# ethz-asl/multipoint

Measured on AMD Instinct MI355X. Metric: image-pairs/sec (detect+desc+match) @ 480x640, higher is better.
Workload: dtype f32

## Files before the change

multipoint_amd/csrc/conv_wino43.hip:

```cpp
#include "mp_common.h"
#include "mp_device.h"
#include "mp_tile.h"

#include <algorithm>
#include <type_traits>

MP_TIMING_TABLE(g_timing_q, 256 * 8, mp_debug_read_timing_wino43)
MP_TIMING_HEIGHT(g_timing_q_sel, 480, mp_debug_select_height_wino43)

namespace {

constexpr int NPIX = 18 * 34;
constexpr int UC4 = 4;
constexpr int VB4 = UC4 * 32 * 36;
constexpr int UB4 = UC4 * 64 * 36;
constexpr int NRB = (NPIX + 63) / 64;
constexpr int RB4 = NRB * 64 * 4;
constexpr int SW4 = 8 * 36 * 2;


template <int LEAD = 0>
__device__ __forceinline__ void dma16(const float* sbase, unsigned voff_bytes, unsigned lds_byte)
{
    lds_dma<4, LEAD, 0>(sbase, voff_bytes, lds_byte);
}

template <bool POOL, bool BNF, int TC4, bool F1, bool SPLIT = false, bool VIN = false>
__global__ __launch_bounds__(512, 2) void conv_wino43_kernel(const ConvParams p)
{
    static_assert(!(F1 && SPLIT), "the fused first block is never split");
    static_assert(!(VIN && (F1 || SPLIT)), "pre-transformed input: plain launches only");
    constexpr int TR4 = 32 / TC4;
    constexpr int OY = 4 * TR4, OX = 4 * TC4;
    constexpr int PY = OY + 2, PX = OX + 2;
    static_assert(PY * PX == NPIX, "item shape");
    __shared__ __attribute__((aligned(16))) float Vs[(VIN ? 4 : 2) * VB4];
    __shared__ __attribute__((aligned(16))) float Us[2 * UB4];
    __shared__ __attribute__((aligned(16))) float raw[VIN ? 256 : 3 * RB4 + 256];
    __shared__ __attribute__((aligned(16))) float scr[VIN ? 4 : 8 * SW4];
    __shared__ __attribute__((aligned(16))) float prm[(POOL && !SPLIT ? 6 : 3) * 64];

    const int tid = threadIdx.x;
    const int lane = tid & 63;
    const int wave = __builtin_amdgcn_readfirstlane(tid >> 6);
    const int tb = wave & 1, cb = wave >> 1;
    const int NC = SPLIT ? (p.cin / UC4) >> p.ks_shift : p.cin / UC4;

    const XcdRange xr = xcd_range(p.nitems, p.xcd_shift);
    const int stride = xr.stride, item_end = xr.item_end;
    int item = xr.item;
    if (item >= item_end) return;

    struct Where { int slice, img, y0, x0, tile; const float* in_base; };
    auto decode = [&](int it) __attribute__((always_inline)) -> Where {
        Where w{};
        const int tile = (int)udiv((unsigned)it, p.magic_slices, (unsigned)p.nslices);
        w.slice = it - tile * p.nslices;
        w.tile = tile;
        const int trow = (int)udiv((unsigned)tile, p.magic_tx, (unsigned)p.tiles_x);
        const int tx = tile - trow * p.tiles_x;
        const int bi = (int)udiv((unsigned)trow, p.magic_ty, (unsigned)p.tiles_y);
        const int ty = trow - bi * p.tiles_y;
        w.img = p.img_list ? p.img_list[bi] : bi;
        w.y0 = ty * OY; w.x0 = tx * OX;
        w.in_base = p.in_planar ? p.in + (long long)w.img * (p.cin / 4) * p.H * p.W * 4
                                : p.in + (long long)w.img * p.H * p.W * p.in_cstride + p.in_coff;
        if constexpr (SPLIT)
            w.in_base += (long long)((w.slice & ((1 << p.ks_shift) - 1)) * NC) * (p.in_planar ? (long long)p.H * p.W * 4 : UC4);
        return w;
    };

    const int pix_stride = p.in_planar ? 4 : p.in_cstride;
    const long long unit_stride = p.in_planar ? (long long)p.H * p.W * 4 : UC4;
    const int x_shift = p.in_planar == MP_LAYOUT_XPLANAR ? 2 : 0, x_mask = p.in_planar == MP_LAYOUT_XPLANAR ? 3 : 0;
    const int row_stride = p.W * pix_stride;
    auto pixel_off = [&](int y, int x) __attribute__((always_inline)) -> int {
        return y * row_stride + (x >> x_shift) * pix_stride + (x & x_mask) * p.W;
    };
    unsigned rvoff[2];
    bool roff_rel = false;
    auto raw_offsets = [&](const Where& w) __attribute__((always_inline)) -> const float* {
        const bool interior = (w.y0 >= 1) && (w.y0 + OY < p.H) && (w.x0 >= 1) && (w.x0 + OX < p.W);
        if (interior) {
            if (!roff_rel) {
#pragma unroll
                for (int j = 0; j < 2; ++j) {
                    const int f = (wave + 8 * j) * 64 + lane;
                    const int py = f / PX, px = f - py * PX;
                    rvoff[j] = (f < NPIX) ? (unsigned)pixel_off(py, px + x_mask) * 4u : 0u;
                }
                roff_rel = true;
            }
            return w.in_base + pixel_off(w.y0 - 1, w.x0 - 1 - x_mask);
        }
        roff_rel = false;
#pragma unroll
        for (int j = 0; j < 2; ++j) {
            const int f = (wave + 8 * j) * 64 + lane;
            const int py = f / PX, px = f - py * PX;
            unsigned off = 0;
            if (f < NPIX) {
                const int gy = reflect_clamp(w.y0 + py - 1, p.H), gx = reflect_clamp(w.x0 + px - 1, p.W);
                off = (unsigned)pixel_off(gy, gx) * 4u;
            }
            rvoff[j] = off;
        }
        return w.in_base;
    };
    const unsigned raw_lds = lds_addr(raw), us_lds = lds_addr(Us);
    const unsigned raw_m0 = raw_lds + (unsigned)wave * 1024u;
    const unsigned raw_dummy = raw_lds + 3u * RB4 * 4u;
    auto raw_dma = [&](const float* src, unsigned boff_bytes, int j) __attribute__((always_inline)) {
        const unsigned dst = j == 0 ? raw_m0 + boff_bytes : (wave + 8 < NRB ? raw_m0 + 8192u + boff_bytes : raw_dummy);
        dma16(src, rvoff[j], dst);
    };
    int u_first, u_cnt;
    if constexpr (F1) {
        constexpr int cnt_[8] = {3, 3, 6, 6, 4, 4, 5, 5}, first_[8] = {0, 3, 14, 20, 6, 10, 26, 31};
        u_cnt = 3; u_first = 0;
#pragma unroll
        for (int w = 0; w < 8; ++w) { u_cnt = wave == w ? cnt_[w] : u_cnt; u_first = wave == w ? first_[w] : u_first; }
    } else {
        u_cnt = wave < 4 ? 5 : 4; u_first = wave < 4 ? 5 * wave : 20 + 4 * (wave - 4);
    }
    auto u_dma_site = [&](const float* ub, int buf, int site) __attribute__((always_inline)) {
        if constexpr (VIN) {
#pragma unroll
            for (int i = 3 * site; i < (site ? 5 : 3); ++i) {
                int b = wave + 8 * i;
                b = b < 36 ? b : 35;
                dma16(ub + b * 256, (unsigned)lane * 16u, us_lds + (unsigned)(buf * UB4 + b * 256) * 4u);
            }
            return;
        }
#pragma unroll
        for (int k = 3 * site; k < 3 * site + 3; ++k)
            if (k < u_cnt) {
                const int b = u_first + k;
                dma16<1>(ub + b * 256, (unsigned)lane * 16u, us_lds + (unsigned)(buf * UB4 + b * 256) * 4u);
            }
    };
    auto u_ptr = [&](int slice) __attribute__((always_inline)) -> const float* {
        return p.wpack + (long long)slice * NC * UB4;
    };
    auto load_prm = [&](int vslice) __attribute__((always_inline)) {
        const int slice = SPLIT ? vslice >> p.ks_shift : vslice;
        if (tid < 64) {
            const float sc = p.scale[slice * 64 + tid];
            prm[tid] = p.bias[slice * 64 + tid]; prm[128 + tid] = p.shift[slice * 64 + tid];
            if constexpr (POOL && !SPLIT) {
                const bool neg = sc < 0.f;
                prm[64 + tid] = fabsf(sc); prm[192 + tid] = neg ? -1.f : 1.f;
                prm[256 + tid] = __int_as_float(neg ? (int)0x80000000 : 0); prm[320 + tid] = __int_as_float(neg ? 0 : 0x7fffffff);
            } else {
                prm[64 + tid] = sc;
            }
        }
    };

    const int win = tid >> 3, sub = tid & 7;
    const int w_tile = win >> 1, w_cp = win & 1;
    const int w_ty = w_tile / TC4, w_tx = w_tile % TC4;
    const int sub6 = sub < 6 ? sub : 5;
    const int p1_read = ((4 * w_ty) * PX + 4 * w_tx + sub6) * 4 + 2 * w_cp;
    float* const myscr = scr + wave * SW4 + (win & 7) * 72;
    const unsigned scr_w = lds_addr(myscr + sub6 * 2);
    const int p2_write = (2 * w_cp * 32 + w_tile) * 36 + 6 * sub6;
    f32x2 td[6], tr[6];
    typedef const __attribute__((address_space(3))) f32x2* lds_pair_ptr;
    const unsigned p1_base = lds_addr(raw) + (unsigned)p1_read * 4u;
    unsigned p1_a = p1_base, p1_b = p1_base + 4u * PX * 16u;
    auto tf_pass1 = [&]() __attribute__((always_inline)) {
#pragma unroll
        for (int i = 0; i < 4; ++i) td[i] = reinterpret_cast<lds_pair_ptr>(p1_a)[i * PX * 2];
#pragma unroll
        for (int i = 4; i < 6; ++i) td[i] = reinterpret_cast<lds_pair_ptr>(p1_b)[(i - 4) * PX * 2];
    };
    auto tf_pass1b = [&](unsigned next_byte) __attribute__((always_inline)) {
        bt6(td, tr);
        p1_a = p1_base + next_byte; p1_b = p1_base + 4u * PX * 16u + next_byte;
    };
    auto tf_pass1w = [&](int k) __attribute__((always_inline)) {
        unsigned long long save;
        if (k == 0)
            asm volatile("s_mov_b64 %0, exec\n\ts_and_b64 exec, exec, %4\n\tds_write2_b64 %1, %2, %3 offset0:0 offset1:6\n\ts_mov_b64 exec, %0"
                         : "=&s"(save) : "v"(scr_w), "v"(tr[0]), "v"(tr[1]), "s"(0x3F3F3F3F3F3F3F3Full) : "memory");
        else if (k == 1)
            asm volatile("s_mov_b64 %0, exec\n\ts_and_b64 exec, exec, %4\n\tds_write2_b64 %1, %2, %3 offset0:12 offset1:18\n\ts_mov_b64 exec, %0"
                         : "=&s"(save) : "v"(scr_w), "v"(tr[2]), "v"(tr[3]), "s"(0x3F3F3F3F3F3F3F3Full) : "memory");
        else
            asm volatile("s_mov_b64 %0, exec\n\ts_and_b64 exec, exec, %4\n\tds_write2_b64 %1, %2, %3 offset0:24 offset1:30\n\ts_mov_b64 exec, %0"
                         : "=&s"(save) : "v"(scr_w), "v"(tr[4]), "v"(tr[5]), "s"(0x3F3F3F3F3F3F3F3Full) : "memory");
    };
    auto tf_pass2 = [&]() __attribute__((always_inline)) {
#pragma unroll
        for (int j = 0; j < 6; ++j) td[j] = *reinterpret_cast<const f32x2*>(&myscr[(sub6 * 6 + j) * 2]);
    };
    const unsigned p2_addr = lds_addr(Vs) + (unsigned)p2_write * 4u;
    auto tf_pass2b = [&]() __attribute__((always_inline)) {
        bt6(td, tr);
    };
    auto tf_pass2w = [&](int buf, int k) __attribute__((always_inline)) {
        const unsigned a0 = p2_addr + (unsigned)buf * (VB4 * 4u), a1 = a0 + 32u * 36u * 4u;
        const int j = 2 * k;
        unsigned long long save;
#define MPQ_VST(O0, O1)                                                                                                        \
        asm volatile("s_mov_b64 %0, exec\n\ts_and_b64 exec, exec, %7\n\tds_write2_b32 %1, %2, %3 offset0:" #O0 " offset1:" #O1   \
                     "\n\tds_write2_b32 %4, %5, %6 offset0:" #O0 " offset1:" #O1 "\n\ts_mov_b64 exec, %0"                        \
                     : "=&s"(save) : "v"(a0), "v"(tr[j][0]), "v"(tr[j + 1][0]), "v"(a1), "v"(tr[j][1]), "v"(tr[j + 1][1]),       \
                       "s"(0x3F3F3F3F3F3F3F3Full) : "memory")
        if (k == 0) MPQ_VST(0, 1);
        else if (k == 1) MPQ_VST(2, 3);
        else MPQ_VST(4, 5);
#undef MPQ_VST
    };

    const int a_base = ((lane >> 4) * 64 + cb * 16 + (lane & 15)) * 36;
    const int b_base = ((lane >> 4) * 32 + tb * 16 + (lane & 15)) * 36;
    f32x4 af[3], bf[3];

    constexpr int IW1 = PX + 2, IH1 = PY + 2;
    constexpr int IPB = 768;
    static_assert(!F1 || (IH1 * IW1 <= IPB && 2 * IPB + 16 * 4 + 16 * 4 * 12 <= RB4), "F1: patches + parameters + weights must fit the third raw buffer");
    const unsigned ip_lds = raw_lds + 2u * RB4 * 4u;
    const unsigned bst_lds = ip_lds + 2u * IPB * 4u;
    const unsigned w1_lds = bst_lds + 16u * 4u * 4u;
    typedef const __attribute__((address_space(3))) float* lds_f32_ptr;
    typedef const __attribute__((address_space(3))) f32x4* lds_f32x4_ptr;
    typedef __attribute__((address_space(3))) f32x4* lds_f32x4_wptr;
    unsigned pg_x[2] = {0u, 0u}, pg_w[2] = {0u, 0u};
    bool pg_rel = false;
    int pc_par = 0;
    auto prod_offsets = [&](const Where& w) __attribute__((always_inline)) {
        const bool interior = (w.y0 >= 1) && (w.y0 + OY < p.H) && (w.x0 >= 1) && (w.x0 + OX < p.W);
#pragma unroll
        for (int j = 0; j < 2; ++j) {
            const int f = (wave + 8 * j) * 64 + lane;
            const int fc = f < NPIX ? f : NPIX - 1;
            const int py = fc / PX, px = fc - py * PX;
            int oy = py, ox = px;
            if (!interior) {
                oy = reflect_clamp(w.y0 + py - 1, p.H) - w.y0 + 1; ox = reflect_clamp(w.x0 + px - 1, p.W) - w.x0 + 1;
                oy = min(max(oy, 0), IH1 - 3); ox = min(max(ox, 0), IW1 - 3);
            }
            pg_x[j] = ip_lds + (unsigned)(pc_par * IPB + oy * IW1 + ox) * 4u;
            pg_w[j] = (unsigned)f * 16u;
        }
        pg_rel = interior;
    };
    auto patch_dma = [&](const Where& w, int par) __attribute__((always_inline)) {
        const float* const im = p.img + (long long)w.img * p.H * p.W;
#pragma unroll
        for (int j = 0; j < 2; ++j) {
            if (wave * 64 + 512 * j >= IH1 * IW1) continue;
            const int q = min(tid + 512 * j, IH1 * IW1 - 1);
            const int r = q / IW1, c = q - r * IW1;
            const unsigned off = (unsigned)(reflect_clamp(w.y0 - 2 + r, p.H) * p.W + reflect_clamp(w.x0 - 2 + c, p.W)) * 4u;
            lds_dma<1, 0, 0>(im, off, ip_lds + (unsigned)(par * IPB + wave * 64 + 512 * j) * 4u);
        }
    };
    int pc_unit = 0, pc_next_item = item + stride;
    unsigned pc_wv = w1_lds + (unsigned)(lane & 3) * 48u;
    unsigned pc_bv = bst_lds;
    float px_[9];
    f32x4 pw_[3], pd_;
    auto gather_x = [&](float (&x)[9], const int j) __attribute__((always_inline)) {
        const lds_f32_ptr xp = reinterpret_cast<lds_f32_ptr>(pg_x[j]);
#pragma unroll
        for (int t = 0; t < 9; ++t) x[t] = xp[(t / 3) * IW1 + (t % 3)];
    };
    auto prod_step = [&](const int k, const unsigned wbuf, const int j, const float (&x)[9]) __attribute__((always_inline)) {
        const lds_f32x4_ptr wp = reinterpret_cast<lds_f32x4_ptr>(pc_wv);
        const lds_f32x4_ptr bp = reinterpret_cast<lds_f32x4_ptr>(pc_bv);
        if (k == 0) {
            pd_ = bp[0];
            pw_[0] = wp[0]; pw_[1] = wp[1]; pw_[2] = wp[2];
        } else if (k <= 9) {
            pd_ = __builtin_amdgcn_mfma_f32_4x4x1f32(pw_[(k - 1) >> 2][(k - 1) & 3], x[k - 1], pd_, 0, 0, 0);
        } else {
            const f32x4 v = {relu_bits(pd_[0]), relu_bits(pd_[1]), relu_bits(pd_[2]), relu_bits(pd_[3])};
            *reinterpret_cast<lds_f32x4_wptr>(raw_lds + wbuf + pg_w[j]) = v;
        }
    };
    auto produce = [&](const unsigned wbuf, const int j) __attribute__((always_inline)) {
        if (j == 0) {
#pragma unroll
            for (int k = 0; k <= 10; ++k) prod_step(k, wbuf, 0, px_);
        } else {
            float qx[9];
            gather_x(qx, 1);
#pragma unroll
            for (int k = 0; k <= 10; ++k) prod_step(k, wbuf, 1, qx);
        }
    };
    auto prod_advance = [&]() __attribute__((always_inline)) {
        pc_wv += 4u * 12u * 4u; pc_bv += 4u * 4u;
        if (++pc_unit == NC) {
            pc_unit = 0;
            pc_wv -= (unsigned)NC * 4u * 12u * 4u; pc_bv -= (unsigned)NC * 4u * 4u;
            if (pc_next_item < item_end) {
                const Where w = decode(pc_next_item);
                pc_par ^= 1;
                if (!(pg_rel && (w.y0 >= 1) && (w.y0 + OY < p.H) && (w.x0 >= 1) && (w.x0 + OX < p.W))) prod_offsets(w);
                else {
                    const unsigned flip = pc_par ? (unsigned)IPB * 4u : 0u - (unsigned)IPB * 4u;
                    pg_x[0] += flip; pg_x[1] += flip;
                }
                gather_x(px_, 0);
                pc_next_item += stride;
            }
        }
    };

    const unsigned vs_lds = lds_addr(Vs);
    auto v_dma = [&](const float* vsrc, int slot, int i) __attribute__((always_inline)) {
        const int b = wave + 8 * i;
        const unsigned dst = b < 18 ? vs_lds + (unsigned)(slot * VB4 + b * 256) * 4u : lds_addr(raw);
        dma16(vsrc + (b < 18 ? b : 17) * 256, (unsigned)lane * 16u, dst);
    };
    const float* vcur = nullptr;
    int v_chunk = 0, v_next_item = item + stride;
    auto v_advance = [&]() __attribute__((always_inline)) {
        vcur += VB4;
        if (++v_chunk == NC) {
            v_chunk = 0;
            if (v_next_item < item_end) {
                vcur = p.vglobal + (long long)decode(v_next_item).tile * NC * VB4;
                v_next_item += stride;
            } else {
                vcur -= (long long)NC * VB4;
            }
        }
    };

    Where cur = decode(item);
    if constexpr (F1) {
        for (int f = tid; f < 16 * 4 * 12; f += 512) {
            const int ch = f / 12, t = f - ch * 12;
            (raw + 2 * RB4 + 2 * IPB + 16 * 4)[f] = t < 9 ? p.w1[t * 64 + ch] : 0.f;
        }
        if (tid < 64) (raw + 2 * RB4 + 2 * IPB)[tid] = p.b1[tid];
        patch_dma(cur, 0);
        if (item + stride < item_end) patch_dma(decode(item + stride), 1);
        prod_offsets(cur);
        dma_wait();
        __syncthreads();
        gather_x(px_, 0);
        produce(0u, 0); if (wave + 8 < NRB) produce(0u, 1);
        prod_advance();
        produce(RB4 * 4u, 0); if (wave + 8 < NRB) produce(RB4 * 4u, 1);
        prod_advance();
    }
    const float* rbase = (F1 || VIN) ? p.in : raw_offsets(cur);
    const float* rsrc = rbase;
    Where ld_item = cur;
    int ld_chunk = 0;
    int ld_next_item = item + stride;
    auto ld_advance = [&]() __attribute__((always_inline)) {
        rsrc += unit_stride;
        if (++ld_chunk == NC) {
            ld_chunk = 0;
            if (ld_next_item < item_end) {
                ld_item = decode(ld_next_item);
                rbase = raw_offsets(ld_item);
                ld_next_item += stride;
            }
            rsrc = rbase;
        }
    };
    const float* up = u_ptr(cur.slice);
    if constexpr (VIN) {
        vcur = p.vglobal + (long long)cur.tile * NC * VB4;
#pragma unroll
        for (int u = 0; u < 3; ++u) {
            v_dma(vcur, u, 0); v_dma(vcur, u, 1); v_dma(vcur, u, 2);
            v_advance();
        }
    } else if constexpr (!F1) {
        raw_dma(rsrc, 0u, 0); raw_dma(rsrc, 0u, 1); ld_advance();
        raw_dma(rsrc, RB4 * 4u, 0); raw_dma(rsrc, RB4 * 4u, 1); ld_advance();
        raw_dma(rsrc, 2u * RB4 * 4u, 0); raw_dma(rsrc, 2u * RB4 * 4u, 1); ld_advance();
    }
    unsigned rd_byte = 0u, rt_byte = RB4 * 4u;
    u_dma_site(up, 0, 0); u_dma_site(up, 0, 1);
    u_dma_site(up + UB4, 1, 0); u_dma_site(up + UB4, 1, 1);
    load_prm(cur.slice);
    dma_wait();
    __syncthreads();
    if constexpr (!VIN) {
        tf_pass1(); tf_pass1b(RB4 * 4u); tf_pass1w(0); tf_pass1w(1); tf_pass1w(2); tf_pass2(); tf_pass2b();
        tf_pass2w(0, 0); tf_pass2w(0, 1); tf_pass2w(0, 2);
        asm volatile("s_waitcnt lgkmcnt(0)" ::: "memory");
        __syncthreads();
    }
    af[0] = *reinterpret_cast<const f32x4*>(&Us[a_base]);
    bf[0] = *reinterpret_cast<const f32x4*>(&Vs[b_base]);
    af[1] = *reinterpret_cast<const f32x4*>(&Us[a_base + 4]);
    bf[1] = *reinterpret_cast<const f32x4*>(&Vs[b_base + 4]);

    const f32x4 zero4 = {0.f, 0.f, 0.f, 0.f};
    int cur_par = 0;
#ifdef MP_TIMING
    unsigned long long tsum[8] = {0, 0, 0, 0, 0, 0, 0, 0};
    const bool t_on = ((POOL ? p.H : -p.H) == g_timing_q_sel);
#endif
    for (;;) {
        MP_CLOCK(t_item);
        f32x4 acc[36];
        const int item_next = item + stride;
        const bool has_next = item_next < item_end;
        const int next_slice = has_next ? (int)(item_next - (int)udiv((unsigned)item_next, p.magic_slices, (unsigned)p.nslices) * p.nslices)
                                        : cur.slice;
        const float* unext = u_ptr(next_slice);
        auto tf_at = [&](const int g, const int e, const int vb) __attribute__((always_inline)) {
            constexpr int S[2][8][2] = {
                {{0, 2}, {2, 2}, {2, 3}, {3, 1}, {3, 2}, {5, 2}, {5, 3}, {6, 1}},
                {{0, 2}, {2, 2}, {2, 3}, {3, 1}, {3, 2}, {4, 3}, {5, 1}, {6, 1}}};
            constexpr int TFS = (TC4 == 8 && !F1) ? 1 : 0;
            auto at = [&](const int k) { return g == S[TFS][k][0] && e == S[TFS][k][1]; };
            if (at(0)) tf_pass1();
            if (at(1)) { tf_pass1b(F1 ? (unsigned)vb * (RB4 * 4u) : 3u * RB4 * 4u - rd_byte - rt_byte); tf_pass1w(0); }
            if (at(2)) tf_pass1w(1);
            if (at(3)) tf_pass1w(2);
            if (at(4)) tf_pass2();
            if (at(5)) { tf_pass2b(); tf_pass2w(vb ^ 1, 0); }
            if (at(6)) tf_pass2w(vb ^ 1, 1);
            if (at(7)) tf_pass2w(vb ^ 1, 2);
        };
        auto prod_at = [&](const int g, const int e, const int vb) __attribute__((always_inline)) {
            const unsigned wbuf = (unsigned)vb * (RB4 * 4u);
            constexpr int slot_g[11] = {0, 0, 1, 1, 1, 2, 3, 4, 4, 4, 5};
            constexpr int slot_e[11] = {1, 3, 1, 2, 3, 1, 3, 1, 2, 3, 1};
            if (g == 0 && e == 0) { if (wave + 8 < NRB) produce(wbuf, 1); }
#pragma unroll
            for (int k = 0; k <= 10; ++k)
                if (g == slot_g[k] && e == slot_e[k]) prod_step(k, wbuf, 0, px_);
        };
        auto unit_body = [&](const int c, auto first_tag, auto vb_tag, auto vs_tag) __attribute__((always_inline)) {
            constexpr bool FIRST = decltype(first_tag)::value;
            constexpr int vb = decltype(vb_tag)::value;
            constexpr int vs = VIN ? decltype(vs_tag)::value : vb;
            constexpr int vsn = VIN ? (vs + 1) & 3 : vb ^ 1;
            const float* const ur = Us + vb * UB4 + a_base;
            const float* const vr = Vs + vs * VB4 + b_base;
            const float* const urn = Us + (vb ^ 1) * UB4 + a_base;
            const float* const vrn = Vs + vsn * VB4 + b_base;
            const float* const un2 = c + 2 < NC ? up + (long long)(c + 2) * UB4 : unext + (long long)(c + 2 - NC) * UB4;
            MP_CLOCK(t_u0);
#ifdef MP_TIMING
            unsigned long long t_b0 = 0, t_b1 = 0;
#endif
#pragma unroll
            for (int g = 0; g < 9; ++g) {
#pragma unroll
                for (int e = 0; e < 4; ++e) {
                    const int s = 4 * g + e;
                    acc[s] = __builtin_amdgcn_mfma_f32_16x16x4f32(af[g % 3][e], bf[g % 3][e], FIRST ? zero4 : acc[s], 0, 0, 0);
                    __builtin_amdgcn_sched_barrier(0);
                    if constexpr (!VIN) { if (e != 2) tf_at(g, e, vb); }
                    if constexpr (F1) prod_at(g, e, vb);
                    if (e == 0) {
                        af[(g + 2) % 3] = *reinterpret_cast<const f32x4*>(g + 2 < 9 ? &ur[4 * (g + 2)] : &urn[4 * (g - 7)]);
                        bf[(g + 2) % 3] = *reinterpret_cast<const f32x4*>(g + 2 < 9 ? &vr[4 * (g + 2)] : &vrn[4 * (g - 7)]);
                    } else if (e == 1) {
                        if (g == 7) u_dma_site(un2, vb, 0);
                        else if (g == 8) u_dma_site(un2, vb, 1);
                        else if (g == 0) { if constexpr (VIN) v_dma(vcur, (vs + 3) & 3, 0); else if constexpr (!F1) raw_dma(rsrc, rd_byte, 0); }
                        else if (g == 1) { if constexpr (VIN) v_dma(vcur, (vs + 3) & 3, 1); else if constexpr (!F1) raw_dma(rsrc, rd_byte, 1); }
                        else if (g == 2) { if constexpr (VIN) v_dma(vcur, (vs + 3) & 3, 2); }
                    } else if (e == 2) {
                        if constexpr (!VIN) tf_at(g, 2, vb);
                    } else {
                        if (g == 6) {
#ifdef MP_TIMING
                            t_b0 = __builtin_amdgcn_s_memtime();
#endif
                            if constexpr (F1) asm volatile("s_waitcnt vmcnt(0) lgkmcnt(0)" ::: "memory");
                            else if constexpr (VIN) asm volatile("s_waitcnt vmcnt(3) lgkmcnt(0)" ::: "memory");
                            else asm volatile("s_waitcnt vmcnt(2) lgkmcnt(0)" ::: "memory");
#ifdef MP_TIMING
                            t_b1 = __builtin_amdgcn_s_memtime();
#endif
                            __syncthreads();
#ifdef MP_TIMING
                            tsum[4] += __builtin_amdgcn_s_memtime() - t_b1;
#endif
                        }
                    }
                    __builtin_amdgcn_sched_barrier(0);
                }
            }
            MP_CLOCK(t_u1);
            MP_CLOCK_ADD(0, t_u0, t_u1);
            MP_CLOCK_ADD(1, t_b0, t_b1);
        };
        auto unit = [&](const int c, auto first_tag, auto vb_tag, auto vs_tag) __attribute__((always_inline)) {
            unit_body(c, first_tag, vb_tag, vs_tag);
            if constexpr (VIN) {
                v_advance();
            } else if constexpr (F1) {
                prod_advance();
            } else {
                ld_advance();
                const unsigned ro = 3u * RB4 * 4u - rd_byte - rt_byte;
                rd_byte = rt_byte; rt_byte = ro;
            }
        };
        using VB0 = std::integral_constant<int, 0>;
        using VB1 = std::integral_constant<int, 1>;
        using VS2 = std::integral_constant<int, 2>;
        using VS3 = std::integral_constant<int, 3>;
        if constexpr (VIN) {
            unit(0, std::true_type{}, VB0{}, VB0{});
            for (int c = 1; c + 3 < NC; c += 4) {
                unit(c, std::false_type{}, VB1{}, VB1{});
                unit(c + 1, std::false_type{}, VB0{}, VS2{});
                unit(c + 2, std::false_type{}, VB1{}, VS3{});
                unit(c + 3, std::false_type{}, VB0{}, VB0{});
            }
            unit(NC - 3, std::false_type{}, VB1{}, VB1{});
            unit(NC - 2, std::false_type{}, VB0{}, VS2{});
            unit(NC - 1, std::false_type{}, VB1{}, VS3{});
        } else {
        unit(0, std::true_type{}, VB0{}, VB0{});
        for (int c = 1; c + 1 < NC; c += 2) {
            unit(c, std::false_type{}, VB1{}, VB1{});
            unit(c + 1, std::false_type{}, VB0{}, VB0{});
        }
        unit(NC - 1, std::false_type{}, VB1{}, VB1{});
        }

        MP_CLOCK(t_e0);
        MP_CLOCK_ADD(3, t_item, t_e0);
        if constexpr (F1) { if (item_next + stride < item_end) patch_dma(decode(item_next + stride), cur_par); }
        const int tl = tb * 16 + (lane & 15);
        const int cl = cb * 16 + 4 * (lane >> 4);
        const f32x4 b4 = *reinterpret_cast<const f32x4*>(&prm[cl]);
        const f32x4 s4 = *reinterpret_cast<const f32x4*>(&prm[64 + cl]);
        const f32x4 t4 = *reinterpret_cast<const f32x4*>(&prm[128 + cl]);
        const int oy = cur.y0 + 4 * (tl / TC4), ox = cur.x0 + 4 * (tl % TC4);
        const int ch0 = (SPLIT ? cur.slice >> p.ks_shift : cur.slice) * 64 + cl;
        const int cs = p.out_cstride;
        constexpr int NO = POOL ? 2 : 4;
        f32x2 keep[NO][NO];
        if constexpr (SPLIT) {
            unsigned long long* const part = reinterpret_cast<unsigned long long*>(p.split_scratch) + (long long)item * (2 * 16 * 512) + tid;
#pragma unroll
            for (int h = 0; h < 2; ++h) {
                f32x2 tcol[4][6];
#pragma unroll
                for (int j = 0; j < 6; ++j) {
                    f32x2 m[6], y[4];
#pragma unroll
                    for (int i = 0; i < 6; ++i) m[i] = f32x2{acc[6 * i + j][2 * h], acc[6 * i + j][2 * h + 1]};
                    at6s(m, y);
#pragma unroll
                    for (int a = 0; a < 4; ++a) tcol[a][j] = y[a];
                }
#pragma unroll
                for (int a = 0; a < 4; ++a) {
                    f32x2 y[4];
                    at6s(tcol[a], y);
#pragma unroll
                    for (int b = 0; b < 4; ++b)
                        part[(h * 16 + a * 4 + b) * 512] = __builtin_bit_cast(unsigned long long, y[b]);
                }
            }
        }
        if constexpr (!SPLIT) {
#pragma unroll
        for (int h = 0; h < 2; ++h) {
            f32x2 tcol[4][6];
            if constexpr (!SPLIT) {
#pragma unroll
            for (int j = 0; j < 6; ++j) {
                f32x2 m[6], y[4];
#pragma unroll
                for (int i = 0; i < 6; ++i) m[i] = f32x2{acc[6 * i + j][2 * h], acc[6 * i + j][2 * h + 1]};
                at6s(m, y);
#pragma unroll
                for (int a = 0; a < 4; ++a) tcol[a][j] = y[a];
            }
            }
            const f32x2 bb = {b4[2 * h], b4[2 * h + 1]}, ss = {s4[2 * h], s4[2 * h + 1]}, tt = {t4[2 * h], t4[2 * h + 1]};
            f32x2 res[NO][NO];
            if constexpr (POOL) {
                const f32x4 g4 = *reinterpret_cast<const f32x4*>(&prm[192 + cl]);
                const f32x4 lo4 = *reinterpret_cast<const f32x4*>(&prm[256 + cl]), hi4 = *reinterpret_cast<const f32x4*>(&prm[320 + cl]);
                const f32x2 gg = {g4[2 * h], g4[2 * h + 1]};
                const f32x2 gb = bb * gg;
                constexpr float A1 = (float)MP_W43_A, A2 = A1 * A1, A3 = A2 * A1, A4 = A2 * A2;
                const f32x2 gk[5] = {gg, gg * f32x2{A1, A1}, gg * f32x2{A2, A2}, gg * f32x2{A3, A3}, gg * f32x2{A4, A4}};
                f32x2 xv[4][4];
#pragma unroll
                for (int a = 0; a < 4; ++a) {
                    f32x2 y[4];
                    at6s(tcol[a], y);
#pragma unroll
                    for (int b = 0; b < 4; ++b) {
                        const int e = (a == 1 ? 1 : a == 2 ? 2 : 0) + (b == 1 ? 1 : b == 2 ? 2 : 0);
                        xv[a][b] = __builtin_elementwise_fma(y[b], gk[e], gb);
                    }
                }
#pragma unroll
                for (int a = 0; a < NO; ++a)
#pragma unroll
                    for (int b = 0; b < NO; ++b) {
                        f32x2 m;
#pragma unroll
                        for (int r = 0; r < 2; ++r)
                            m[r] = fmaxf(fmaxf(xv[2 * a][2 * b][r], xv[2 * a][2 * b + 1][r]), fmaxf(xv[2 * a + 1][2 * b][r], xv[2 * a + 1][2 * b + 1][r]));
                        if (BNF) {
                            m = __builtin_elementwise_fma(m, ss, tt);
                            m = f32x2{relu_bits(m[0]), relu_bits(m[1])};
                        } else {
#pragma unroll
                            for (int r = 0; r < 2; ++r)
                                asm("v_med3_i32 %0, %1, %2, %3" : "=v"(m[r]) : "v"(m[r]), "v"(lo4[2 * h + r]), "v"(hi4[2 * h + r]));
                            m = __builtin_elementwise_fma(m, ss, tt);
                        }
                        res[a][b] = m;
                    }
            } else {
            f32x2 yv[4][4];
#pragma unroll
            for (int a = 0; a < 4; ++a) {
                f32x2 y[4];
                at6s(tcol[a], y);
#pragma unroll
                for (int b = 0; b < 4; ++b) {
                    f32x2 v = w43_add_bias(y[b], a, b, bb);
                    if (BNF) { v = v * ss + tt; v = f32x2{relu_bits(v[0]), relu_bits(v[1])}; }
                    else { v = f32x2{relu_bits(v[0]), relu_bits(v[1])}; v = v * ss + tt; }
                    yv[a][b] = v;
                }
            }
#pragma unroll
            for (int a = 0; a < NO; ++a)
#pragma unroll
                for (int b = 0; b < NO; ++b) res[a][b] = yv[a][b];
            }
            if (h == 0) {
#pragma unroll
                for (int a = 0; a < NO; ++a)
#pragma unroll
                    for (int b = 0; b < NO; ++b) keep[a][b] = res[a][b];
            } else {
                const int Ho = POOL ? p.H >> 1 : p.H, Wo = POOL ? p.W >> 1 : p.W;
                const int py0 = POOL ? oy >> 1 : oy, px0 = POOL ? ox >> 1 : ox;
                const bool xpl = !POOL && p.out_planar == MP_LAYOUT_XPLANAR;
                char* const img_base = reinterpret_cast<char*>(
                    p.out_planar ? p.out + (long long)cur.img * (p.cout / 4) * Ho * Wo * 4
                                 : p.out + (long long)cur.img * Ho * Wo * cs + p.out_coff);
                const unsigned ps = xpl ? (unsigned)Wo * 4u : p.out_planar ? 16u : (unsigned)cs * 4u;
                const unsigned rs = p.out_planar ? (unsigned)Wo * 16u : (unsigned)Wo * ps;
                const unsigned o0 = xpl ? (unsigned)(((ch0 >> 2) * Ho + py0) * Wo * 4 + px0) * 4u
                                  : p.out_planar ? (unsigned)(((ch0 >> 2) * Ho + py0) * Wo + px0) * 16u
                                                 : (unsigned)((py0 * Wo + px0) * cs + ch0) * 4u;
                if (oy < p.H && ox < p.W && ch0 < p.cout) {
#pragma unroll
                    for (int a = 0; a < NO; ++a)
#pragma unroll
                        for (int b = 0; b < NO; ++b) {
                            const f32x4 v = {keep[a][b][0], keep[a][b][1], res[a][b][0], res[a][b][1]};
                            *reinterpret_cast<f32x4*>(img_base + (o0 + (unsigned)a * rs + (unsigned)b * ps)) = v;
                        }
                }
            }
        }
        }
        MP_CLOCK(t_e1);
        MP_CLOCK_ADD(2, t_e0, t_e1);
#ifdef MP_TIMING
        tsum[7] += 1;
        if (!has_next && tid == 0 && t_on)
            for (int i = 0; i < 8; ++i) g_timing_q[blockIdx.x * 8 + i] = tsum[i];
#endif
        if (!has_next) { dma_wait(); return; }
        if (next_slice != cur.slice) {
            __syncthreads();
            load_prm(next_slice);
        }
        item = item_next;
        cur = decode(item);
        cur_par ^= 1;
        up = unext;
    }
}

template <int TC4>
__global__ __launch_bounds__(256) void wino43_vprod_kernel(const ConvParams p, long long ntb)
{
    constexpr int TR4 = 32 / TC4, OY = 4 * TR4, OX = 4 * TC4;
    __shared__ __attribute__((aligned(16))) float st[19456];
    const int ncp = p.cin >> 1, NC = p.cin / UC4;
    const int TL = 256 / ncp;
    const int RS = TL * 36 + 4;
    const int groups = 32 / TL;
    const int tid = threadIdx.x;
    const int cp = tid % ncp, tlc = tid / ncp;
    const long long tb = (long long)blockIdx.x / groups;
    const int t0 = ((int)((long long)blockIdx.x % groups)) * TL, t = t0 + tlc;
    (void)ntb;
    const int tx = (int)(tb % p.tiles_x);
    const long long trow = tb / p.tiles_x;
    const int ty = (int)(trow % p.tiles_y);
    const int bi = (int)(trow / p.tiles_y);
    const int img = p.img_list ? p.img_list[bi] : bi;
    const int wy = ty * OY + 4 * (t / TC4) - 1, wx = tx * OX + 4 * (t % TC4) - 1;
    const float* const base = p.in + (long long)img * p.H * p.W * p.in_cstride + p.in_coff + 2 * cp;
    int gx[6];
#pragma unroll
    for (int j = 0; j < 6; ++j) gx[j] = reflect_clamp(wx + j, p.W);
    f32x2 r[6][6];
#pragma unroll
    for (int j = 0; j < 6; ++j) {
        f32x2 d[6], o[6];
#pragma unroll
        for (int i = 0; i < 6; ++i)
            d[i] = *reinterpret_cast<const f32x2*>(base + ((long long)reflect_clamp(wy + i, p.H) * p.W + gx[j]) * p.in_cstride);
        bt6(d, o);
#pragma unroll
        for (int i = 0; i < 6; ++i) r[i][j] = o[i];
    }
    float* const dst0 = st + (2 * cp) * RS + tlc * 36;
    float* const dst1 = dst0 + RS;
#pragma unroll
    for (int i = 0; i < 6; i += 2) {
        f32x2 a[6], b[6];
        bt6(r[i], a);
        bt6(r[i + 1], b);
        *reinterpret_cast<f32x4*>(dst0 + 6 * i) = f32x4{a[0][0], a[1][0], a[2][0], a[3][0]};
        *reinterpret_cast<f32x4*>(dst0 + 6 * i + 4) = f32x4{a[4][0], a[5][0], b[0][0], b[1][0]};
        *reinterpret_cast<f32x4*>(dst0 + 6 * i + 8) = f32x4{b[2][0], b[3][0], b[4][0], b[5][0]};
        *reinterpret_cast<f32x4*>(dst1 + 6 * i) = f32x4{a[0][1], a[1][1], a[2][1], a[3][1]};
        *reinterpret_cast<f32x4*>(dst1 + 6 * i + 4) = f32x4{a[4][1], a[5][1], b[0][1], b[1][1]};
        *reinterpret_cast<f32x4*>(dst1 + 6 * i + 8) = f32x4{b[2][1], b[3][1], b[4][1], b[5][1]};
    }
    __syncthreads();
    const int q4 = TL * 9, total4 = p.cin * q4;
    float* const gbase = p.vglobal + (tb * NC * 4 * 32 + t0) * 36;
    for (int i = tid; i < total4; i += 256) {
        const int row = i / q4, w = i - row * q4;
        *reinterpret_cast<f32x4*>(gbase + (long long)row * (32 * 36) + w * 4) = *reinterpret_cast<const f32x4*>(st + row * RS + w * 4);
    }
}

template <bool POOL, int TC4, bool F1 = false, bool SPLIT = false>
int launch_q(const ConvParams& p, hipStream_t s)
{
    constexpr int OY = 4 * (32 / TC4), OX = 4 * TC4;
    ConvParams q = p;
    if (SPLIT) q.nslices = p.nslices << p.ks_shift;
    q.tiles_x = (p.W + OX - 1) / OX; q.tiles_y = (p.H + OY - 1) / OY;
    const long long nitems = (long long)p.B * q.tiles_x * q.tiles_y * q.nslices;
    if (nitems <= 0) return 0;
    if (tile_items(q, nitems)) return 1;
    const unsigned grid = persistent_grid(nitems, p.ncu, p.xcd_shift);
    const ConvParams& pp = q;
    if (p.bn_first) hipLaunchKernelGGL((conv_wino43_kernel<POOL, true, TC4, F1, SPLIT>), dim3(grid), dim3(512), 0, s, pp);
    else hipLaunchKernelGGL((conv_wino43_kernel<POOL, false, TC4, F1, SPLIT>), dim3(grid), dim3(512), 0, s, pp);
    return 0;
}

template <int TC4>
int launch_vin(const ConvParams& p, hipStream_t s)
{
    constexpr int OY = 4 * (32 / TC4), OX = 4 * TC4;
    ConvParams q = p;
    q.tiles_x = (p.W + OX - 1) / OX; q.tiles_y = (p.H + OY - 1) / OY;
    const long long ntb = (long long)p.B * q.tiles_x * q.tiles_y, nitems = ntb * q.nslices;
    if (nitems <= 0) return 0;
    if (tile_items(q, nitems)) return 1;
    const ConvParams& pp = q;
    const int tl = 256 / (p.cin / 2);
    hipLaunchKernelGGL((wino43_vprod_kernel<TC4>), dim3((unsigned)(ntb * (32 / tl))), dim3(256), 0, s, pp, ntb);
    const unsigned grid = persistent_grid(nitems, p.ncu, p.xcd_shift);
    if (p.bn_first) hipLaunchKernelGGL((conv_wino43_kernel<false, true, TC4, false, false, true>), dim3(grid), dim3(512), 0, s, pp);
    else hipLaunchKernelGGL((conv_wino43_kernel<false, false, TC4, false, false, true>), dim3(grid), dim3(512), 0, s, pp);
    return 0;
}

template <bool POOL, bool SPLIT = false>
int launch_shape(const ConvParams& p, hipStream_t s)
{
    const long long wide = (long long)((p.W + 31) / 32) * ((p.H + 15) / 16), tall = (long long)((p.W + 15) / 16) * ((p.H + 31) / 32);
    return tall < wide ? launch_q<POOL, 4, false, SPLIT>(p, s) : launch_q<POOL, 8, false, SPLIT>(p, s);
}

}

bool conv_wino43_supports(const ConvParams& p)
{
    return !p.pad_zero && p.cin % 8 == 0 && p.cout % 4 == 0 && p.H % 4 == 0 && p.W % 4 == 0 && p.H >= 4 && p.W >= 4 &&
           p.in_cstride % 4 == 0 && p.in_coff % 4 == 0 && p.out_cstride % 4 == 0 && p.out_coff % 4 == 0;
}

long long conv_wino43_vglobal_floats(const ConvParams& p)
{
    const long long wide = (long long)((p.W + 31) / 32) * ((p.H + 15) / 16), tall = (long long)((p.W + 15) / 16) * ((p.H + 31) / 32);
    return (long long)p.B * std::min(wide, tall) * (p.cin / UC4) * VB4;
}

long long conv_wino43_items(const ConvParams& p)
{
    const long long wide = (long long)((p.W + 31) / 32) * ((p.H + 15) / 16), tall = (long long)((p.W + 15) / 16) * ((p.H + 31) / 32);
    return (long long)p.B * std::min(wide, tall) * p.nslices;
}

int launch_conv_wino43(const ConvParams& p, bool pool, hipStream_t s, bool fuse_first)
{
    if (p.out_planar == MP_LAYOUT_XPLANAR && pool) return 2;
    if ((p.in_planar == MP_LAYOUT_XPLANAR || p.out_planar == MP_LAYOUT_XPLANAR) && p.ks_shift > 0) return 2;
    if (fuse_first) return pool && p.cin == 64 ? launch_q<true, 8, true>(p, s) : 2;
    if (p.vglobal) {
        if (pool || p.ks_shift > 0 || p.cin % 16 != 0 || p.in_planar || p.cin > 256 || 256 % (p.cin / 2) != 0 || (p.cin / 2) < 8) return 2;
        const long long wide = (long long)((p.W + 31) / 32) * ((p.H + 15) / 16), tall = (long long)((p.W + 15) / 16) * ((p.H + 31) / 32);
        return tall < wide ? launch_vin<4>(p, s) : launch_vin<8>(p, s);
    }
    if (p.ks_shift > 0) {
        const int ncs = (p.cin / 4) >> p.ks_shift;
        if (ncs < 4 || (ncs & 1) || (ncs << p.ks_shift) * 4 != p.cin || !p.split_scratch) return 2;
        const int rc = pool ? launch_shape<true, true>(p, s) : launch_shape<false, true>(p, s);
        return rc ? rc : launch_split_reduce(p, 1, pool, s);
    }
    return pool ? launch_shape<true>(p, s) : launch_shape<false>(p, s);
}
```

Before: 3473.

## Broadcast first-layer conv weights via MFMA blocks and share bias across pixel groups

Repacks the first-layer 3x3 weights so each lane holds a single scalar. The 4x4x1 MFMA block-broadcast modifier selects the tap weight per step, which replaces the previous three f32x4 weight registers per lane. The second pixel group is now produced from the same loaded bias accumulator, and its patch gather is hoisted into the item-advance point instead of being done inside produce. It also drops the F1-specific uneven weight-DMA split between waves and adds asm barriers to keep indexing from being folded. The intent is to cut VGPR pressure and LDS weight reads in the fused producer, at the cost of keeping nine more live patch values (qx_) and relying on broadcast semantics being correct.

```diff
diff --git a/multipoint_amd/csrc/conv_wino43.hip b/multipoint_amd/csrc/conv_wino43.hip
--- a/multipoint_amd/csrc/conv_wino43.hip
+++ b/multipoint_amd/csrc/conv_wino43.hip
@@ -114,15 +114,7 @@
         const unsigned dst = j == 0 ? raw_m0 + boff_bytes : (wave + 8 < NRB ? raw_m0 + 8192u + boff_bytes : raw_dummy);
         dma16(src, rvoff[j], dst);
     };
-    int u_first, u_cnt;
-    if constexpr (F1) {
-        constexpr int cnt_[8] = {3, 3, 6, 6, 4, 4, 5, 5}, first_[8] = {0, 3, 14, 20, 6, 10, 26, 31};
-        u_cnt = 3; u_first = 0;
-#pragma unroll
-        for (int w = 0; w < 8; ++w) { u_cnt = wave == w ? cnt_[w] : u_cnt; u_first = wave == w ? first_[w] : u_first; }
-    } else {
-        u_cnt = wave < 4 ? 5 : 4; u_first = wave < 4 ? 5 * wave : 20 + 4 * (wave - 4);
-    }
+    const int u_cnt = wave < 4 ? 5 : 4, u_first = wave < 4 ? 5 * wave : 20 + 4 * (wave - 4);
     auto u_dma_site = [&](const float* ub, int buf, int site) __attribute__((always_inline)) {
         if constexpr (VIN) {
 #pragma unroll
@@ -146,14 +138,16 @@
     auto load_prm = [&](int vslice) __attribute__((always_inline)) {
         const int slice = SPLIT ? vslice >> p.ks_shift : vslice;
         if (tid < 64) {
-            const float sc = p.scale[slice * 64 + tid];
-            prm[tid] = p.bias[slice * 64 + tid]; prm[128 + tid] = p.shift[slice * 64 + tid];
+            int t = tid;
+            if constexpr (F1) asm volatile("" : "+v"(t));
+            const float sc = p.scale[slice * 64 + t];
+            prm[t] = p.bias[slice * 64 + t]; prm[128 + t] = p.shift[slice * 64 + t];
             if constexpr (POOL && !SPLIT) {
                 const bool neg = sc < 0.f;
-                prm[64 + tid] = fabsf(sc); prm[192 + tid] = neg ? -1.f : 1.f;
-                prm[256 + tid] = __int_as_float(neg ? (int)0x80000000 : 0); prm[320 + tid] = __int_as_float(neg ? 0 : 0x7fffffff);
+                prm[64 + t] = fabsf(sc); prm[192 + t] = neg ? -1.f : 1.f;
+                prm[256 + t] = __int_as_float(neg ? (int)0x80000000 : 0); prm[320 + t] = __int_as_float(neg ? 0 : 0x7fffffff);
             } else {
-                prm[64 + tid] = sc;
+                prm[64 + t] = sc;
             }
         }
     };
@@ -221,7 +215,7 @@
 
     constexpr int IW1 = PX + 2, IH1 = PY + 2;
     constexpr int IPB = 768;
-    static_assert(!F1 || (IH1 * IW1 <= IPB && 2 * IPB + 16 * 4 + 16 * 4 * 12 <= RB4), "F1: patches + parameters + weights must fit the third raw buffer");
+    static_assert(!F1 || (IH1 * IW1 <= IPB && 2 * IPB + 16 * 4 + 16 * 48 <= RB4), "F1: patches + parameters + weights must fit the third raw buffer");
     const unsigned ip_lds = raw_lds + 2u * RB4 * 4u;
     const unsigned bst_lds = ip_lds + 2u * IPB * 4u;
     const unsigned w1_lds = bst_lds + 16u * 4u * 4u;
@@ -253,51 +247,67 @@
 #pragma unroll
         for (int j = 0; j < 2; ++j) {
             if (wave * 64 + 512 * j >= IH1 * IW1) continue;
-            const int q = min(tid + 512 * j, IH1 * IW1 - 1);
+            int q = tid + 512 * j;
+            asm volatile("" : "+v"(q));
+            q = min(q, IH1 * IW1 - 1);
             const int r = q / IW1, c = q - r * IW1;
             const unsigned off = (unsigned)(reflect_clamp(w.y0 - 2 + r, p.H) * p.W + reflect_clamp(w.x0 - 2 + c, p.W)) * 4u;
             lds_dma<1, 0, 0>(im, off, ip_lds + (unsigned)(par * IPB + wave * 64 + 512 * j) * 4u);
         }
     };
     int pc_unit = 0, pc_next_item = item + stride;
-    unsigned pc_wv = w1_lds + (unsigned)(lane & 3) * 48u;
+    unsigned pc_wv = w1_lds + (unsigned)min(lane, 47) * 4u;
     unsigned pc_bv = bst_lds;
-    float px_[9];
-    f32x4 pw_[3], pd_;
+    float px_[9], qx_[9];
+    float pw_;
+    f32x4 pd_;
     auto gather_x = [&](float (&x)[9], const int j) __attribute__((always_inline)) {
         const lds_f32_ptr xp = reinterpret_cast<lds_f32_ptr>(pg_x[j]);
 #pragma unroll
         for (int t = 0; t < 9; ++t) x[t] = xp[(t / 3) * IW1 + (t % 3)];
     };
-    auto prod_step = [&](const int k, const unsigned wbuf, const int j, const float (&x)[9]) __attribute__((always_inline)) {
-        const lds_f32x4_ptr wp = reinterpret_cast<lds_f32x4_ptr>(pc_wv);
-        const lds_f32x4_ptr bp = reinterpret_cast<lds_f32x4_ptr>(pc_bv);
+    auto tap_mfma = [&](const int t, const float x, const f32x4 c) __attribute__((always_inline)) -> f32x4 {
+        switch (t) {
+        case 0: return __builtin_amdgcn_mfma_f32_4x4x1f32(pw_, x, c, 4, 0, 0);
+        case 1: return __builtin_amdgcn_mfma_f32_4x4x1f32(pw_, x, c, 4, 1, 0);
+        case 2: return __builtin_amdgcn_mfma_f32_4x4x1f32(pw_, x, c, 4, 2, 0);
+        case 3: return __builtin_amdgcn_mfma_f32_4x4x1f32(pw_, x, c, 4, 3, 0);
+        case 4: return __builtin_amdgcn_mfma_f32_4x4x1f32(pw_, x, c, 4, 4, 0);
+        case 5: return __builtin_amdgcn_mfma_f32_4x4x1f32(pw_, x, c, 4, 5, 0);
+        case 6: return __builtin_amdgcn_mfma_f32_4x4x1f32(pw_, x, c, 4, 6, 0);
+        case 7: return __builtin_amdgcn_mfma_f32_4x4x1f32(pw_, x, c, 4, 7, 0);
+        default: return __builtin_amdgcn_mfma_f32_4x4x1f32(pw_, x, c, 4, 8, 0);
+        }
+    };
+    auto prod_step = [&](const int k, const unsigned wbuf) __attribute__((always_inline)) {
         if (k == 0) {
-            pd_ = bp[0];
-            pw_[0] = wp[0]; pw_[1] = wp[1]; pw_[2] = wp[2];
+            pd_ = reinterpret_cast<lds_f32x4_ptr>(pc_bv)[0];
+            pw_ = reinterpret_cast<lds_f32_ptr>(pc_wv)[0];
         } else if (k <= 9) {
-            pd_ = __builtin_amdgcn_mfma_f32_4x4x1f32(pw_[(k - 1) >> 2][(k - 1) & 3], x[k - 1], pd_, 0, 0, 0);
+            pd_ = tap_mfma(k - 1, px_[k - 1], pd_);
         } else {
             const f32x4 v = {relu_bits(pd_[0]), relu_bits(pd_[1]), relu_bits(pd_[2]), relu_bits(pd_[3])};
-            *reinterpret_cast<lds_f32x4_wptr>(raw_lds + wbuf + pg_w[j]) = v;
-        }
-    };
-    auto produce = [&](const unsigned wbuf, const int j) __attribute__((always_inline)) {
-        if (j == 0) {
-#pragma unroll
-            for (int k = 0; k <= 10; ++k) prod_step(k, wbuf, 0, px_);
-        } else {
-            float qx[9];
-            gather_x(qx, 1);
-#pragma unroll
-            for (int k = 0; k <= 10; ++k) prod_step(k, wbuf, 1, qx);
-        }
+            *reinterpret_cast<lds_f32x4_wptr>(raw_lds + wbuf + pg_w[0]) = v;
+        }
+    };
+    auto produce2 = [&](const unsigned wbuf) __attribute__((always_inline)) {
+        f32x4 d = tap_mfma(0, qx_[0], pd_);
+#pragma unroll
+        for (int t = 1; t < 9; ++t) d = tap_mfma(t, qx_[t], d);
+        const f32x4 v = {relu_bits(d[0]), relu_bits(d[1]), relu_bits(d[2]), relu_bits(d[3])};
+        *reinterpret_cast<lds_f32x4_wptr>(raw_lds + wbuf + pg_w[1]) = v;
+    };
+    auto produce = [&](const unsigned wbuf) __attribute__((always_inline)) {
+        prod_step(0, wbuf);
+        if (wave + 8 < NRB) produce2(wbuf);
+#pragma unroll
+        for (int k = 1; k <= 10; ++k) prod_step(k, wbuf);
     };
     auto prod_advance = [&]() __attribute__((always_inline)) {
-        pc_wv += 4u * 12u * 4u; pc_bv += 4u * 4u;
+        pc_wv += 48u * 4u; pc_bv += 4u * 4u;
         if (++pc_unit == NC) {
             pc_unit = 0;
-            pc_wv -= (unsigned)NC * 4u * 12u * 4u; pc_bv -= (unsigned)NC * 4u * 4u;
+            pc_wv -= (unsigned)NC * 48u * 4u; pc_bv -= (unsigned)NC * 4u * 4u;
             if (pc_next_item < item_end) {
                 const Where w = decode(pc_next_item);
                 pc_par ^= 1;
@@ -307,6 +317,7 @@
                     pg_x[0] += flip; pg_x[1] += flip;
                 }
                 gather_x(px_, 0);
+                if (wave + 8 < NRB) gather_x(qx_, 1);
                 pc_next_item += stride;
             }
         }
@@ -335,9 +346,9 @@
 
     Where cur = decode(item);
     if constexpr (F1) {
-        for (int f = tid; f < 16 * 4 * 12; f += 512) {
-            const int ch = f / 12, t = f - ch * 12;
-            (raw + 2 * RB4 + 2 * IPB + 16 * 4)[f] = t < 9 ? p.w1[t * 64 + ch] : 0.f;
+        for (int f = tid; f < 16 * 48; f += 512) {
+            const int u = f / 48, l = f - u * 48;
+            (raw + 2 * RB4 + 2 * IPB + 16 * 4)[f] = l < 36 ? p.w1[(l >> 2) * 64 + 4 * u + (l & 3)] : 0.f;
         }
         if (tid < 64) (raw + 2 * RB4 + 2 * IPB)[tid] = p.b1[tid];
         patch_dma(cur, 0);
@@ -346,9 +357,10 @@
         dma_wait();
         __syncthreads();
         gather_x(px_, 0);
-        produce(0u, 0); if (wave + 8 < NRB) produce(0u, 1);
+        if (wave + 8 < NRB) gather_x(qx_, 1);
+        produce(0u);
         prod_advance();
-        produce(RB4 * 4u, 0); if (wave + 8 < NRB) produce(RB4 * 4u, 1);
+        produce(RB4 * 4u);
         prod_advance();
     }
     const float* rbase = (F1 || VIN) ? p.in : raw_offsets(cur);
@@ -430,11 +442,11 @@
         auto prod_at = [&](const int g, const int e, const int vb) __attribute__((always_inline)) {
             const unsigned wbuf = (unsigned)vb * (RB4 * 4u);
             constexpr int slot_g[11] = {0, 0, 1, 1, 1, 2, 3, 4, 4, 4, 5};
-            constexpr int slot_e[11] = {1, 3, 1, 2, 3, 1, 3, 1, 2, 3, 1};
-            if (g == 0 && e == 0) { if (wave + 8 < NRB) produce(wbuf, 1); }
+            constexpr int slot_e[11] = {0, 3, 1, 2, 3, 1, 3, 1, 2, 3, 1};
 #pragma unroll
             for (int k = 0; k <= 10; ++k)
-                if (g == slot_g[k] && e == slot_e[k]) prod_step(k, wbuf, 0, px_);
+                if (g == slot_g[k] && e == slot_e[k]) prod_step(k, wbuf);
+            if (g == 0 && e == 0) { if (wave + 8 < NRB) produce2(wbuf); }
         };
         auto unit_body = [&](const int c, auto first_tag, auto vb_tag, auto vs_tag) __attribute__((always_inline)) {
             constexpr bool FIRST = decltype(first_tag)::value;
```

New measurement: 3533, median of 6. 1.02x the previous value.
